# constantinpape/torch-em

Measured on AMD Instinct MI355X. Metric: voxels/sec fwd+bwd, UNet3d 1x128^3 bs=2, higher is better.
Workload: dtype f32-class (forward convs on normalised activations: fp32 operands split into 2 fp16 terms = 22 mantissa bits, lo plane scaled by 2^12 with its own fp32 accumulator, 3 fp16 MFMAs per product; other forward convs 3 bf16 terms / 6 MFMAs; data-gradient convs 2 bf16 terms / 3 MFMAs (16-bit products); WEI

## Files before the change

### torch_em_amd/csrc/conv1x1_stream.hip

```cpp
#include "tem_common.h"
#include "tem_act.h"
#include "conv_split.h"
#include "conv_internal.h"
#include "conv_arith.h"

template <int NS, bool F16, int CT, typename T>
__global__ __launch_bounds__(256) void k_conv1x1_stream(const T* __restrict__ x, int64_t x_ld,
                                                        const unsigned short* __restrict__ wp,
                                                        const float* __restrict__ bias, T* __restrict__ y,
                                                        int64_t y_ld, const T* __restrict__ ref, int64_t ref_ld,
                                                        int64_t NV, int Cin, int Cout, int act, int64_t nmt,
                                                        unsigned* __restrict__ amax) {
    const int lane = threadIdx.x & 63, wv = threadIdx.x >> 6;
    float amx = 0.f;
    const int r = lane & 31, kh = lane >> 5;
    const int ctg = blockIdx.y;
    const int nks = Cin >> 4;
    const uint4* wfrag = reinterpret_cast<const uint4*>(wp) + lane;
    for (int64_t mt = (int64_t)blockIdx.x * 4 + wv; mt < nmt; mt += (int64_t)gridDim.x * 4) {
        const int64_t v = mt * 32 + r;
        const bool vok = v < NV;
        const T* xr = x + (vok ? v : 0) * x_ld + kh * 8;
        floatx16 acc[CT];
#pragma unroll
        for (int ct = 0; ct < CT; ++ct)
#pragma unroll
            for (int k = 0; k < 16; ++k) acc[ct][k] = 0.f;
        for (int ks = 0; ks < nks; ++ks) {
            uint4 t[NS];
            if constexpr (sizeof(T) == 2) {
                static_assert(sizeof(T) == 4 || NS == 1, "16-bit storage: one-term modes only");
                t[0] = make_uint4(0u, 0u, 0u, 0u);
                if (vok) t[0] = *reinterpret_cast<const uint4*>(xr + ks * 16);
            } else {
                float4 a0 = make_float4(0.f, 0.f, 0.f, 0.f), a1 = a0;
                if (vok) {
                    a0 = act_ld4(xr + ks * 16);
                    a1 = act_ld4(xr + ks * 16 + 4);
                }
                float rem[8] = {a0.x, a0.y, a0.z, a0.w, a1.x, a1.y, a1.z, a1.w};
#pragma unroll
                for (int p = 0; p < NS; ++p) {
                    unsigned wds[4];
#pragma unroll
                    for (int e = 0; e < 4; ++e) {
                        const unsigned h = pk16<F16>(rem[2 * e], rem[2 * e + 1]);
                        wds[e] = h;
                        if (p + 1 < NS) {
                            rem[2 * e] -= lo16<F16>(h);
                            rem[2 * e + 1] -= hi16<F16>(h);
                        }
                    }
                    t[p] = make_uint4(wds[0], wds[1], wds[2], wds[3]);
                }
            }
#pragma unroll
            for (int ct = 0; ct < CT; ++ct) {
                const int nt = ctg * CT + ct;
                if (nt * 32 < Cout) {
                    const uint4* f = wfrag + ((int64_t)(nt * nks + ks) * NS) * 64;
                    uint4 b[NS];
#pragma unroll
                    for (int p = 0; p < NS; ++p) b[p] = f[p * 64];
#pragma unroll
                    for (int o = NS - 1; o >= 0; --o)
#pragma unroll
                        for (int i = 0; i <= o; ++i) acc[ct] = mfma16<F16>(b[o - i], t[i], acc[ct]);
                }
            }
        }
        if (vok) {
#pragma unroll
            for (int ct = 0; ct < CT; ++ct) {
#pragma unroll
                for (int q4 = 0; q4 < 4; ++q4) {
                    const int co = (ctg * CT + ct) * 32 + 8 * q4 + 4 * kh;
                    if (co < Cout) {
                        float4 o = make_float4(acc[ct][4 * q4], acc[ct][4 * q4 + 1], acc[ct][4 * q4 + 2], acc[ct][4 * q4 + 3]);
                        if (bias) {
                            const float4 b4 = *reinterpret_cast<const float4*>(bias + co);
                            o.x += b4.x;
                            o.y += b4.y;
                            o.z += b4.z;
                            o.w += b4.w;
                        }
                        o.x = act_apply_b(o.x, act);
                        o.y = act_apply_b(o.y, act);
                        o.z = act_apply_b(o.z, act);
                        o.w = act_apply_b(o.w, act);
                        if (ref) {
                            const float4 rv = act_ld4(ref + v * ref_ld + co);
                            o.x = rv.x > 0.f ? o.x : 0.f;
                            o.y = rv.y > 0.f ? o.y : 0.f;
                            o.z = rv.z > 0.f ? o.z : 0.f;
                            o.w = rv.w > 0.f ? o.w : 0.f;
                        }
                        act_st4(y + v * y_ld + co, o);
                        amx = tem_amax4(amx, o.x, o.y, o.z, o.w);
                    }
                }
            }
        }
    }
    if (amax) tem_amax_commit(amax, amx);
}

template <int NS, bool F16, typename T>
static void stream_launch(const TemConvCall& c, const T* x, int64_t x_ld, const float* wp, const float* bias, T* y, int64_t y_ld,
                          const T* ref, int64_t ref_ld, int64_t NV, int Cin, int Cout, int act, hipStream_t s) {
    const int64_t nmt = (NV + 31) / 32;
    const int ntile = Cout / 32;
    const int CT = ntile >= 2 ? 2 : 1;
    const int ngroups = (ntile + CT - 1) / CT;
    int64_t gx = (nmt + 3) / 4;
    if (gx > 8192) gx = 8192;
    const dim3 grid((unsigned)gx, (unsigned)ngroups);
    unsigned* const amax = c.take_output_amax();
    if (CT == 2)
        hipLaunchKernelGGL((k_conv1x1_stream<NS, F16, 2, T>), grid, dim3(256), 0, s, x, x_ld, (const unsigned short*)wp, bias, y, y_ld,
                           ref, ref_ld, NV, Cin, Cout, act, nmt, amax);
    else
        hipLaunchKernelGGL((k_conv1x1_stream<NS, F16, 1, T>), grid, dim3(256), 0, s, x, x_ld, (const unsigned short*)wp, bias, y, y_ld,
                           ref, ref_ld, NV, Cin, Cout, act, nmt, amax);
}

void tem_conv1x1_stream(const TemConvCall& c, const float* x, int64_t x_ld, const float* wp, const float* bias, float* y, int64_t y_ld,
                        const float* ref, int64_t ref_ld, const TemConvShape& sh, int act, int mode, hipStream_t s) {
    const int st = c.stx, Cin = sh.Cin, Cout = sh.Cout;
    const int64_t NV = sh.NV();
    auto go = [&](auto ns, auto f16, auto t) {
        using T = decltype(t);
        stream_launch<ns(), f16(), T>(c, (const T*)x, x_ld, wp, bias, (T*)y, y_ld, (const T*)ref, ref_ld, NV, Cin, Cout, act, s);
    };
    const TemArith& a = tem_arith(mode);
    if (st == TEM_ST_F16) go(TemInt<1>{}, TemBool<true>{}, tem_f16{});
    else if (st == TEM_ST_BF16) go(TemInt<1>{}, TemBool<false>{}, tem_bf16{});
    else if (a.planes == 3) go(TemInt<3>{}, TemBool<false>{}, float{});
    else if (a.planes == 2) go(TemInt<2>{}, TemBool<false>{}, float{});
    else tem_select_bool(a.elem == TEM_EL_F16, [&](auto f16) { go(TemInt<1>{}, f16, float{}); });
}
```

### torch_em_amd/csrc/dice.hip

```cpp
#include "tem_common.h"

#define DICE_MAX_BLOCKS 2048

extern "C" int64_t tem_dice_ws(int N, int64_t V, int C) {
    (void)N;
    (void)V;
    return (int64_t)DICE_MAX_BLOCKS * C * 4 * (int64_t)sizeof(float);
}

__device__ __forceinline__ float dice_sigmoid(float x) { return 1.f / (1.f + expf(-x)); }

template <bool CFAST>
__global__ void k_dice_partial(const float* __restrict__ p, int64_t p_sn, int64_t p_sc, int64_t p_sv,
                               const float* __restrict__ t, int64_t t_sn, int64_t t_sc, int64_t t_sv,
                               const float* __restrict__ mask, int N, int C, int64_t V, int rows, int64_t vper,
                               int nblk_per_n, float* __restrict__ part, int flags) {
    extern __shared__ float sh[];
    const int NS = (flags & TEM_DICE_BCE) ? 4 : 3;
    const int n = blockIdx.x / nblk_per_n, b = blockIdx.x % nblk_per_n;
    int c, r;
    if (CFAST) {
        c = threadIdx.x % C;
        r = threadIdx.x / C;
    } else {
        r = threadIdx.x % rows;
        c = threadIdx.x / rows;
    }
    int64_t v0 = (int64_t)b * vper, v1 = v0 + vper;
    if (v1 > V) v1 = V;
    const float* pp = p + (int64_t)n * p_sn + (int64_t)c * p_sc;
    const float* tp = t + (int64_t)n * t_sn + (int64_t)c * t_sc;
    const float* mp = mask ? mask + (int64_t)n * t_sn + (int64_t)c * t_sc : nullptr;
    float s0 = 0.f, s1 = 0.f, s2 = 0.f, s3 = 0.f;
    for (int64_t v = v0 + r; v < v1; v += rows) {
        float pv = pp[v * p_sv], tv = tp[v * t_sv];
        if (flags) {
            const float xv = pv;
            if (flags & TEM_DICE_LOGITS) pv = dice_sigmoid(xv);
            if (flags & TEM_DICE_BCE) {
                if (flags & TEM_DICE_LOGITS)
                    s3 += fmaxf(xv, 0.f) - xv * tv + log1pf(expf(-fabsf(xv)));
                else
                    s3 -= tv * fmaxf(logf(pv), -100.f) + (1.f - tv) * fmaxf(logf(1.f - pv), -100.f);
            }
        }
        if (mp) {
            float m = mp[v * t_sv];
            pv *= m;
            tv *= m;
        }
        s0 = fmaf(pv, tv, s0);
        s1 = fmaf(pv, pv, s1);
        s2 = fmaf(tv, tv, s2);
    }
    float* my = sh + ((int64_t)r * C + c) * NS;
    my[0] = s0;
    my[1] = s1;
    my[2] = s2;
    if (NS == 4) my[3] = s3;
    __syncthreads();
    if (r == 0) {
        float a0 = 0.f, a1 = 0.f, a2 = 0.f, a3 = 0.f;
        for (int rr = 0; rr < rows; ++rr) {
            const float* o = sh + ((int64_t)rr * C + c) * NS;
            a0 += o[0];
            a1 += o[1];
            a2 += o[2];
            if (NS == 4) a3 += o[3];
        }
        float* o = part + ((int64_t)blockIdx.x * C + c) * NS;
        o[0] = a0;
        o[1] = a1;
        o[2] = a2;
        if (NS == 4) o[3] = a3;
    }
}

#define DICE_VOX_C 16
template <int VECP>
__global__ __launch_bounds__(256) void k_dice_partial_vox(const float* __restrict__ p, int64_t p_sn, int64_t p_sc, int64_t p_sv,
                                                          const float* __restrict__ t, int64_t t_sn, int64_t t_sc, int64_t t_sv,
                                                          const float* __restrict__ mask, int N, int C, int64_t V, int64_t vper,
                                                          int nblk_per_n, float* __restrict__ part, int flags) {
    __shared__ float shv[4][DICE_VOX_C][4];
    const int NS = (flags & TEM_DICE_BCE) ? 4 : 3;
    const int n = blockIdx.x / nblk_per_n, b = blockIdx.x % nblk_per_n;
    (void)vper;
    const float* pn = p + (int64_t)n * p_sn;
    const float* tn = t + (int64_t)n * t_sn;
    const float* mn = mask ? mask + (int64_t)n * t_sn : nullptr;
    float s0[DICE_VOX_C], s1[DICE_VOX_C], s2[DICE_VOX_C], s3[DICE_VOX_C];
#pragma unroll
    for (int c = 0; c < DICE_VOX_C; ++c) s0[c] = s1[c] = s2[c] = s3[c] = 0.f;
    for (int64_t vb = (int64_t)b * 256 + threadIdx.x; vb < V; vb += (int64_t)nblk_per_n * 256) {
        float pq[DICE_VOX_C], tq[DICE_VOX_C], mq[DICE_VOX_C];
        const float* pv_ = pn + vb * p_sv;
        if constexpr (VECP == 4) {
#pragma unroll
            for (int c = 0; c < DICE_VOX_C; c += 4)
                if (c < C) {
                    const float4 q = *reinterpret_cast<const float4*>(pv_ + c);
                    pq[c] = q.x; pq[c + 1] = q.y; pq[c + 2] = q.z; pq[c + 3] = q.w;
                }
        } else if constexpr (VECP == 2) {
            const float2 q = *reinterpret_cast<const float2*>(pv_);
            pq[0] = q.x; pq[1] = q.y;
        } else {
#pragma unroll
            for (int c = 0; c < DICE_VOX_C; ++c)
                if (c < C) pq[c] = pv_[c * p_sc];
        }
#pragma unroll
        for (int c = 0; c < DICE_VOX_C; ++c)
            if (c < C) {
                tq[c] = tn[c * t_sc + vb * t_sv];
                mq[c] = mn ? mn[c * t_sc + vb * t_sv] : 1.f;
            }
#pragma unroll
        for (int c = 0; c < DICE_VOX_C; ++c)
            if (c < C) {
                float pv = pq[c], tv = tq[c];
                if (flags) {
                    const float xv = pv;
                    if (flags & TEM_DICE_LOGITS) pv = dice_sigmoid(xv);
                    if (flags & TEM_DICE_BCE) {
                        if (flags & TEM_DICE_LOGITS)
                            s3[c] += fmaxf(xv, 0.f) - xv * tv + log1pf(expf(-fabsf(xv)));
                        else
                            s3[c] -= tv * fmaxf(logf(pv), -100.f) + (1.f - tv) * fmaxf(logf(1.f - pv), -100.f);
                    }
                }
                if (mn) {
                    pv *= mq[c];
                    tv *= mq[c];
                }
                s0[c] = fmaf(pv, tv, s0[c]);
                s1[c] = fmaf(pv, pv, s1[c]);
                s2[c] = fmaf(tv, tv, s2[c]);
            }
    }
    const int wv = threadIdx.x >> 6, lane = threadIdx.x & 63;
#pragma unroll
    for (int c = 0; c < DICE_VOX_C; ++c)
        if (c < C) {
            const float a0 = tem_wave_sum(s0[c]), a1 = tem_wave_sum(s1[c]), a2 = tem_wave_sum(s2[c]);
            const float a3 = NS == 4 ? tem_wave_sum(s3[c]) : 0.f;
            if (lane == 0) {
                shv[wv][c][0] = a0;
                shv[wv][c][1] = a1;
                shv[wv][c][2] = a2;
                shv[wv][c][3] = a3;
            }
        }
    __syncthreads();
    for (int i = threadIdx.x; i < C * NS; i += 256) {
        const int c = i / NS, k = i % NS;
        part[((int64_t)blockIdx.x * C + c) * NS + k] = shv[0][c][k] + shv[1][c][k] + shv[2][c][k] + shv[3][c][k];
    }
}

__global__ __launch_bounds__(256) void k_dice_reduce(const float* __restrict__ part, int nblk, int C,
                                                     double* __restrict__ sums, int NS) {
    const int c = blockIdx.x;
    double a[4] = {0.0, 0.0, 0.0, 0.0};
    for (int b = threadIdx.x; b < nblk; b += 256) {
        const float* o = part + ((int64_t)b * C + c) * NS;
        a[0] += (double)o[0];
        a[1] += (double)o[1];
        a[2] += (double)o[2];
        if (NS == 4) a[3] += (double)o[3];
    }
    __shared__ double sh[4][4];
#pragma unroll
    for (int k = 0; k < 4; ++k) {
        a[k] = tem_wave_sum_d(a[k]);
        if ((threadIdx.x & 63) == 0) sh[k][threadIdx.x >> 6] = a[k];
    }
    __syncthreads();
    if (threadIdx.x < NS) sums[c * NS + threadIdx.x] = sh[threadIdx.x][0] + sh[threadIdx.x][1] + sh[threadIdx.x][2] + sh[threadIdx.x][3];
}

static int dice_sums_impl(const float* p, int64_t p_sn, int64_t p_sc, int64_t p_sv, const float* t, int64_t t_sn,
                          int64_t t_sc, int64_t t_sv, const float* mask, int N, int C, int64_t V, double* sums,
                          void* ws, int64_t ws_bytes, int flags, tem_stream_t stream) {
    TEM_REQUIRE(p && t && sums && ws, "tem_dice_sums: null pointer");
    TEM_REQUIRE((flags & ~(TEM_DICE_LOGITS | TEM_DICE_BCE)) == 0 && (!(flags & TEM_DICE_BCE) || !mask),
                "tem_dice_sums2: unknown flags, or the BCE term together with a mask");
    const int NS = (flags & TEM_DICE_BCE) ? 4 : 3;
    TEM_REQUIRE(N > 0 && C > 0 && C <= 1024 && V > 0, "tem_dice_sums: bad shape (C=%d)", C);
    if (ws_bytes < tem_dice_ws(N, V, C)) {
        tem_set_error("tem_dice_sums: workspace too small");
        return TEM_EWS;
    }
    int rows = 256 / C;
    if (rows < 1) rows = 1;
    if (C <= DICE_VOX_C && tem_option(TEM_OPT_DICE_VOX)) rows = 256;
    int threads = C <= DICE_VOX_C && tem_option(TEM_OPT_DICE_VOX) ? 256 : rows * C;
    int64_t nb = tem_cdiv(V, (int64_t)rows * 8);
    int64_t maxb = DICE_MAX_BLOCKS / N;
    if (maxb < 1) {
        tem_set_error("tem_dice_sums: batch too large (N=%d)", N);
        return TEM_EINVAL;
    }
    if (nb > maxb) nb = maxb;
    int64_t vper = tem_cdiv(V, nb);
    int nblk = (int)nb * N;
    size_t lds = (size_t)rows * C * NS * sizeof(float);
    float* part = (float*)ws;
    bool cfast = (p_sc == 1);
    if (C <= DICE_VOX_C && tem_option(TEM_OPT_DICE_VOX)) {
        const bool al = cfast && p_sn % 4 == 0 && p_sv % 4 == 0 && ((uintptr_t)p % 16 == 0);
        if (al && C % 4 == 0)
            hipLaunchKernelGGL((k_dice_partial_vox<4>), dim3(nblk), dim3(256), 0, (hipStream_t)stream, p, p_sn, p_sc, p_sv, t, t_sn,
                               t_sc, t_sv, mask, N, C, V, vper, (int)nb, part, flags);
        else if (cfast && C == 2 && p_sn % 2 == 0 && p_sv == 2 && ((uintptr_t)p % 8 == 0))
            hipLaunchKernelGGL((k_dice_partial_vox<2>), dim3(nblk), dim3(256), 0, (hipStream_t)stream, p, p_sn, p_sc, p_sv, t, t_sn,
                               t_sc, t_sv, mask, N, C, V, vper, (int)nb, part, flags);
        else
            hipLaunchKernelGGL((k_dice_partial_vox<1>), dim3(nblk), dim3(256), 0, (hipStream_t)stream, p, p_sn, p_sc, p_sv, t, t_sn,
                               t_sc, t_sv, mask, N, C, V, vper, (int)nb, part, flags);
    } else if (cfast)
        hipLaunchKernelGGL((k_dice_partial<true>), dim3(nblk), dim3(threads), lds, (hipStream_t)stream, p, p_sn, p_sc,
                           p_sv, t, t_sn, t_sc, t_sv, mask, N, C, V, rows, vper, (int)nb, part, flags);
    else
        hipLaunchKernelGGL((k_dice_partial<false>), dim3(nblk), dim3(threads), lds, (hipStream_t)stream, p, p_sn, p_sc,
                           p_sv, t, t_sn, t_sc, t_sv, mask, N, C, V, rows, vper, (int)nb, part, flags);
    hipLaunchKernelGGL(k_dice_reduce, dim3(C), dim3(256), 0, (hipStream_t)stream, part, nblk, C, sums, NS);
    TEM_CHECK_LAUNCH("tem_dice_sums");
    return TEM_OK;
}

extern "C" int tem_dice_sums(const float* p, int64_t p_sn, int64_t p_sc, int64_t p_sv, const float* t, int64_t t_sn,
                             int64_t t_sc, int64_t t_sv, const float* mask, int N, int C, int64_t V, double* sums,
                             void* ws, int64_t ws_bytes, tem_stream_t stream) {
    return dice_sums_impl(p, p_sn, p_sc, p_sv, t, t_sn, t_sc, t_sv, mask, N, C, V, sums, ws, ws_bytes, 0, stream);
}

extern "C" int tem_dice_sums2(const float* p, int64_t p_sn, int64_t p_sc, int64_t p_sv, const float* t, int64_t t_sn,
                              int64_t t_sc, int64_t t_sv, int N, int C, int64_t V, double* sums, void* ws,
                              int64_t ws_bytes, int flags, tem_stream_t stream) {
    return dice_sums_impl(p, p_sn, p_sc, p_sv, t, t_sn, t_sc, t_sv, nullptr, N, C, V, sums, ws, ws_bytes, flags, stream);
}

__global__ void k_dice_finalize(const double* __restrict__ sums, int C, double eps, int channelwise, int invert,
                                int reduce, float* __restrict__ out, float* __restrict__ ca, float* __restrict__ cb, int NS) {
    if (threadIdx.x != 0 || blockIdx.x != 0) return;
    const double sgn = invert ? -1.0 : 1.0;
    if (!channelwise) {
        double num = 0.0, den = 0.0;
        for (int c = 0; c < C; ++c) {
            num += sums[c * NS];
            den += sums[c * NS + 1] + sums[c * NS + 2];
        }
        double cd = den < eps ? eps : den;
        double score = 2.0 * num / cd;
        out[0] = (float)(invert ? 1.0 - score : score);
        double a = sgn * 2.0 / cd, b = (den >= eps) ? -sgn * 4.0 * num / (cd * cd) : 0.0;
        for (int c = 0; c < C; ++c) {
            ca[c] = (float)a;
            cb[c] = (float)b;
        }
        return;
    }
    double acc = 0.0;
    int arg = 0;
    double best = 0.0;
    for (int c = 0; c < C; ++c) {
        double num = sums[c * NS], den = sums[c * NS + 1] + sums[c * NS + 2];
        double cd = den < eps ? eps : den;
        double score = 2.0 * num / cd;
        double val = invert ? 1.0 - score : score;
        ca[c] = (float)(sgn * 2.0 / cd);
        cb[c] = (float)((den >= eps) ? -sgn * 4.0 * num / (cd * cd) : 0.0);
        if (reduce == 0) out[c] = (float)val;
        acc += val;
        if (c == 0 || (reduce == 3 && val > best) || (reduce == 4 && val < best)) {
            best = val;
            arg = c;
        }
    }
    if (reduce == 1) out[0] = (float)acc;
    if (reduce == 2) {
        out[0] = (float)(acc / C);
        for (int c = 0; c < C; ++c) {
            ca[c] /= (float)C;
            cb[c] /= (float)C;
        }
    }
    if (reduce == 3 || reduce == 4) {
        out[0] = (float)best;
        for (int c = 0; c < C; ++c)
            if (c != arg) {
                ca[c] = 0.f;
                cb[c] = 0.f;
            }
    }
}

static int dice_finalize_impl(const double* sums, int C, double eps, int channelwise, int invert, int reduce, float* out,
                              float* ca, float* cb, int NS, tem_stream_t stream) {
    TEM_REQUIRE(sums && out && ca && cb && C > 0, "tem_dice_finalize: bad arguments");
    TEM_REQUIRE(reduce >= 0 && reduce <= 4, "tem_dice_finalize: Unsupported channel reduction %d", reduce);
    hipLaunchKernelGGL(k_dice_finalize, dim3(1), dim3(64), 0, (hipStream_t)stream, sums, C, eps, channelwise, invert,
                       reduce, out, ca, cb, NS);
    TEM_CHECK_LAUNCH("tem_dice_finalize");
    return TEM_OK;
}
extern "C" int tem_dice_finalize(const double* sums, int C, double eps, int channelwise, int invert, int reduce,
                                 float* out, float* ca, float* cb, tem_stream_t stream) {
    return dice_finalize_impl(sums, C, eps, channelwise, invert, reduce, out, ca, cb, 3, stream);
}
extern "C" int tem_dice_finalize2(const double* sums, int ncol, int C, double eps, int channelwise, int invert, int reduce,
                                  float* out, float* ca, float* cb, tem_stream_t stream) {
    TEM_REQUIRE(ncol == 3 || ncol == 4, "tem_dice_finalize2: ncol must be 3 or 4");
    return dice_finalize_impl(sums, C, eps, channelwise, invert, reduce, out, ca, cb, ncol, stream);
}

template <bool CFAST>
__global__ __launch_bounds__(256) void k_dice_grad(const float* __restrict__ p, int64_t p_sn, int64_t p_sc,
                                                   int64_t p_sv, const float* __restrict__ t, int64_t t_sn,
                                                   int64_t t_sc, int64_t t_sv, const float* __restrict__ mask,
                                                   const float* __restrict__ ca, const float* __restrict__ cb,
                                                   const float* __restrict__ gout, int gout_per_channel,
                                                   float* __restrict__ gp, int64_t g_sn, int64_t g_sc, int64_t g_sv,
                                                   int C, int64_t V, int flags, float w_dice, float w_bce) {
    const int n = blockIdx.y;
    const int64_t items = V * C;
    for (int64_t i = (int64_t)blockIdx.x * 256 + threadIdx.x; i < items; i += (int64_t)gridDim.x * 256) {
        int c;
        int64_t v;
        if (CFAST) {
            v = i / C;
            c = (int)(i - v * C);
        } else {
            c = (int)(i / V);
            v = i - (int64_t)c * V;
        }
        float pv = p[(int64_t)n * p_sn + (int64_t)c * p_sc + v * p_sv];
        float tv = t[(int64_t)n * t_sn + (int64_t)c * t_sc + v * t_sv];
        float m = 1.f;
        if (mask) {
            m = mask[(int64_t)n * t_sn + (int64_t)c * t_sc + v * t_sv];
            pv *= m;
            tv *= m;
        }
        float go = gout ? gout[gout_per_channel ? c : 0] : 1.f;
        if (flags) {
            const float xv = pv;
            if (flags & TEM_DICE_LOGITS) pv = dice_sigmoid(xv);
            float d = w_dice * (ca[c] * tv + cb[c] * pv);
            if (flags & TEM_DICE_LOGITS) d *= pv * (1.f - pv);
            if (flags & TEM_DICE_BCE)
                d += w_bce * ((flags & TEM_DICE_LOGITS) ? (pv - tv) : (pv - tv) / fmaxf(pv * (1.f - pv), 1e-12f));
            gp[(int64_t)n * g_sn + (int64_t)c * g_sc + v * g_sv] = go * d;
            continue;
        }
        gp[(int64_t)n * g_sn + (int64_t)c * g_sc + v * g_sv] = go * (ca[c] * tv + cb[c] * pv) * m;
    }
}

template <int VECP>
__global__ __launch_bounds__(256) void k_dice_grad_vox(const float* __restrict__ p, int64_t p_sn, int64_t p_sc, int64_t p_sv,
                                                       const float* __restrict__ t, int64_t t_sn, int64_t t_sc, int64_t t_sv,
                                                       const float* __restrict__ mask, const float* __restrict__ ca,
                                                       const float* __restrict__ cb, const float* __restrict__ gout,
                                                       int gout_per_channel, float* __restrict__ gp, int64_t g_sn, int64_t g_sc,
                                                       int64_t g_sv, int C, int64_t V, int flags, float w_dice, float w_bce) {
    const int n = blockIdx.y;
    const float* pn = p + (int64_t)n * p_sn;
    const float* tn = t + (int64_t)n * t_sn;
    const float* mn = mask ? mask + (int64_t)n * t_sn : nullptr;
    float* gn = gp + (int64_t)n * g_sn;
    for (int64_t v = (int64_t)blockIdx.x * 256 + threadIdx.x; v < V; v += (int64_t)gridDim.x * 256) {
        float pq[DICE_VOX_C], tq[DICE_VOX_C], mq[DICE_VOX_C], gq[DICE_VOX_C];
        const float* pv_ = pn + v * p_sv;
        if constexpr (VECP == 4) {
#pragma unroll
            for (int c = 0; c < DICE_VOX_C; c += 4)
                if (c < C) {
                    const float4 q = *reinterpret_cast<const float4*>(pv_ + c);
                    pq[c] = q.x; pq[c + 1] = q.y; pq[c + 2] = q.z; pq[c + 3] = q.w;
                }
        } else if constexpr (VECP == 2) {
            const float2 q = *reinterpret_cast<const float2*>(pv_);
            pq[0] = q.x; pq[1] = q.y;
        } else {
#pragma unroll
            for (int c = 0; c < DICE_VOX_C; ++c)
                if (c < C) pq[c] = pv_[c * p_sc];
        }
#pragma unroll
        for (int c = 0; c < DICE_VOX_C; ++c)
            if (c < C) {
                tq[c] = tn[c * t_sc + v * t_sv];
                mq[c] = mn ? mn[c * t_sc + v * t_sv] : 1.f;
            }
#pragma unroll
        for (int c = 0; c < DICE_VOX_C; ++c)
            if (c < C) {
                float pv = pq[c], tv = tq[c];
                const float m = mq[c];
                if (mn) {
                    pv *= m;
                    tv *= m;
                }
                const float go = gout ? gout[gout_per_channel ? c : 0] : 1.f;
                if (flags) {
                    const float xv = pv;
                    if (flags & TEM_DICE_LOGITS) pv = dice_sigmoid(xv);
                    float d = w_dice * (ca[c] * tv + cb[c] * pv);
                    if (flags & TEM_DICE_LOGITS) d *= pv * (1.f - pv);
                    if (flags & TEM_DICE_BCE)
                        d += w_bce * ((flags & TEM_DICE_LOGITS) ? (pv - tv) : (pv - tv) / fmaxf(pv * (1.f - pv), 1e-12f));
                    gq[c] = go * d;
                } else {
                    gq[c] = go * (ca[c] * tv + cb[c] * pv) * m;
                }
            }
        float* gv_ = gn + v * g_sv;
        if constexpr (VECP == 4) {
#pragma unroll
            for (int c = 0; c < DICE_VOX_C; c += 4)
                if (c < C) *reinterpret_cast<float4*>(gv_ + c) = make_float4(gq[c], gq[c + 1], gq[c + 2], gq[c + 3]);
        } else if constexpr (VECP == 2) {
            *reinterpret_cast<float2*>(gv_) = make_float2(gq[0], gq[1]);
        } else {
#pragma unroll
            for (int c = 0; c < DICE_VOX_C; ++c)
                if (c < C) gv_[c * g_sc] = gq[c];
        }
    }
}

static int dice_grad_impl(const float* p, int64_t p_sn, int64_t p_sc, int64_t p_sv, const float* t, int64_t t_sn,
                          int64_t t_sc, int64_t t_sv, const float* mask, const float* ca, const float* cb,
                          const float* gout, int gout_per_channel, float* gp, int64_t g_sn, int64_t g_sc,
                          int64_t g_sv, int N, int C, int64_t V, int flags, float w_dice, float w_bce, tem_stream_t stream) {
    TEM_REQUIRE(p && t && ca && cb && gp && N > 0 && C > 0 && V > 0, "tem_dice_grad: bad arguments");
    TEM_REQUIRE((flags & ~(TEM_DICE_LOGITS | TEM_DICE_BCE)) == 0 && (!flags || !mask), "tem_dice_grad2: unknown flags, or flags with a mask");
    dim3 grid(tem_grid_1d(V * C, 256, 2048), N);
    if (C <= DICE_VOX_C && tem_option(TEM_OPT_DICE_VOX)) {
        const dim3 vgrid(tem_grid_1d(V, 256, 4096), N);
        const bool cl = p_sc == 1 && g_sc == 1;
        const bool al4 = cl && C % 4 == 0 && p_sn % 4 == 0 && p_sv % 4 == 0 && g_sn % 4 == 0 && g_sv % 4 == 0 &&
                         ((uintptr_t)p % 16 == 0) && ((uintptr_t)gp % 16 == 0);
        const bool al2 = cl && C == 2 && p_sv == 2 && g_sv == 2 && p_sn % 2 == 0 && g_sn % 2 == 0 && ((uintptr_t)p % 8 == 0) &&
                         ((uintptr_t)gp % 8 == 0);
#define TEM_DGV(VP)                                                                                                            \
    hipLaunchKernelGGL((k_dice_grad_vox<VP>), vgrid, dim3(256), 0, (hipStream_t)stream, p, p_sn, p_sc, p_sv, t, t_sn, t_sc, t_sv, \
                       mask, ca, cb, gout, gout_per_channel, gp, g_sn, g_sc, g_sv, C, V, flags, w_dice, w_bce)
        if (al4) TEM_DGV(4);
        else if (al2) TEM_DGV(2);
        else TEM_DGV(1);
#undef TEM_DGV
    } else if (p_sc == 1)
        hipLaunchKernelGGL((k_dice_grad<true>), grid, dim3(256), 0, (hipStream_t)stream, p, p_sn, p_sc, p_sv, t, t_sn,
                           t_sc, t_sv, mask, ca, cb, gout, gout_per_channel, gp, g_sn, g_sc, g_sv, C, V, flags, w_dice, w_bce);
    else
        hipLaunchKernelGGL((k_dice_grad<false>), grid, dim3(256), 0, (hipStream_t)stream, p, p_sn, p_sc, p_sv, t, t_sn,
                           t_sc, t_sv, mask, ca, cb, gout, gout_per_channel, gp, g_sn, g_sc, g_sv, C, V, flags, w_dice, w_bce);
    TEM_CHECK_LAUNCH("tem_dice_grad");
    return TEM_OK;
}
extern "C" int tem_dice_grad(const float* p, int64_t p_sn, int64_t p_sc, int64_t p_sv, const float* t, int64_t t_sn,
                             int64_t t_sc, int64_t t_sv, const float* mask, const float* ca, const float* cb,
                             const float* gout, int gout_per_channel, float* gp, int64_t g_sn, int64_t g_sc,
                             int64_t g_sv, int N, int C, int64_t V, tem_stream_t stream) {
    return dice_grad_impl(p, p_sn, p_sc, p_sv, t, t_sn, t_sc, t_sv, mask, ca, cb, gout, gout_per_channel, gp, g_sn, g_sc,
                          g_sv, N, C, V, 0, 1.f, 0.f, stream);
}
extern "C" int tem_dice_grad2(const float* p, int64_t p_sn, int64_t p_sc, int64_t p_sv, const float* t, int64_t t_sn,
                              int64_t t_sc, int64_t t_sv, const float* ca, const float* cb, const float* gout,
                              int gout_per_channel, float* gp, int64_t g_sn, int64_t g_sc, int64_t g_sv, int N, int C,
                              int64_t V, int flags, float w_dice, float w_bce, tem_stream_t stream) {
    return dice_grad_impl(p, p_sn, p_sc, p_sv, t, t_sn, t_sc, t_sv, nullptr, ca, cb, gout, gout_per_channel, gp, g_sn,
                          g_sc, g_sv, N, C, V, flags, w_dice, w_bce, stream);
}
```

Measured before the change: 281.2 million.

## Stage 1x1 conv tiles through LDS with prefetch; unroll dice kernels for C=2

```diff
diff --git a/torch_em_amd/csrc/conv1x1_stream.hip b/torch_em_amd/csrc/conv1x1_stream.hip
--- a/torch_em_amd/csrc/conv1x1_stream.hip
+++ b/torch_em_amd/csrc/conv1x1_stream.hip
@@ -4,81 +4,148 @@
 #include "conv_internal.h"
 #include "conv_arith.h"
 
+#define ST_PITCH 9
+__device__ __forceinline__ void st_lds_fence() { asm volatile("" ::: "memory"); }
+
+struct StLines { uint4 v[4]; };
+template <typename T>
+__device__ __forceinline__ StLines st_load_x(const T* __restrict__ x, int64_t x_ld, int64_t mt, int s, int lr, int lp, int npc, int64_t NV) {
+    StLines o;
+    const int pc = min(s * 8 + lp, npc - 1);
+#pragma unroll
+    for (int j = 0; j < 4; ++j) {
+        const int64_t v = min(mt * 32 + lr + 8 * j, NV - 1);
+        o.v[j] = reinterpret_cast<const uint4*>(x + v * x_ld)[pc];
+    }
+    return o;
+}
+
+template <typename T> struct StRef { typedef act_u2 raw; };
+template <> struct StRef<float> { typedef float4 raw; };
+__device__ __forceinline__ float4 st_ref4(const float*, float4 u) { return u; }
+template <typename T> __device__ __forceinline__ float4 st_ref4(const T*, act_u2 u) {
+    return make_float4(act_lo<T>(u.x), act_hi<T>(u.x), act_lo<T>(u.y), act_hi<T>(u.y));
+}
+
 template <int NS, bool F16, int CT, typename T>
-__global__ __launch_bounds__(256) void k_conv1x1_stream(const T* __restrict__ x, int64_t x_ld,
+__global__ __launch_bounds__(256) __attribute__((amdgpu_waves_per_eu(sizeof(T) == 4 ? 3 : 2))) void k_conv1x1_stream(const T* __restrict__ x, int64_t x_ld,
                                                         const unsigned short* __restrict__ wp,
                                                         const float* __restrict__ bias, T* __restrict__ y,
                                                         int64_t y_ld, const T* __restrict__ ref, int64_t ref_ld,
                                                         int64_t NV, int Cin, int Cout, int act, int64_t nmt,
                                                         unsigned* __restrict__ amax) {
+    static_assert(sizeof(T) == 4 || NS == 1, "16-bit storage: one-term modes only");
+    constexpr int PK = sizeof(T) / 2;
+    constexpr int KPS = 4 / PK;
+    __shared__ uint4 tiles[4][32 * ST_PITCH];
     const int lane = threadIdx.x & 63, wv = threadIdx.x >> 6;
+    uint4* const tl = tiles[wv];
     float amx = 0.f;
     const int r = lane & 31, kh = lane >> 5;
+    const int lr = lane >> 3, lp = lane & 7;
     const int ctg = blockIdx.y;
     const int nks = Cin >> 4;
+    const int npc = nks * 2 * PK;
+    const int nst = (nks + KPS - 1) / KPS;
     const uint4* wfrag = reinterpret_cast<const uint4*>(wp) + lane;
+    float4 bs[CT];
+#pragma unroll
+    for (int ct = 0; ct < CT; ++ct) {
+        const int co = (ctg * CT + ct) * 32 + 4 * lp;
+        bs[ct] = make_float4(0.f, 0.f, 0.f, 0.f);
+        if (bias && co < Cout) bs[ct] = *reinterpret_cast<const float4*>(bias + co);
+    }
     for (int64_t mt = (int64_t)blockIdx.x * 4 + wv; mt < nmt; mt += (int64_t)gridDim.x * 4) {
-        const int64_t v = mt * 32 + r;
-        const bool vok = v < NV;
-        const T* xr = x + (vok ? v : 0) * x_ld + kh * 8;
-        floatx16 acc[CT];
-#pragma unroll
-        for (int ct = 0; ct < CT; ++ct)
-#pragma unroll
-            for (int k = 0; k < 16; ++k) acc[ct][k] = 0.f;
-        for (int ks = 0; ks < nks; ++ks) {
-            uint4 t[NS];
-            if constexpr (sizeof(T) == 2) {
-                static_assert(sizeof(T) == 4 || NS == 1, "16-bit storage: one-term modes only");
-                t[0] = make_uint4(0u, 0u, 0u, 0u);
-                if (vok) t[0] = *reinterpret_cast<const uint4*>(xr + ks * 16);
-            } else {
-                float4 a0 = make_float4(0.f, 0.f, 0.f, 0.f), a1 = a0;
-                if (vok) {
-                    a0 = act_ld4(xr + ks * 16);
-                    a1 = act_ld4(xr + ks * 16 + 4);
-                }
-                float rem[8] = {a0.x, a0.y, a0.z, a0.w, a1.x, a1.y, a1.z, a1.w};
-#pragma unroll
-                for (int p = 0; p < NS; ++p) {
-                    unsigned wds[4];
-#pragma unroll
-                    for (int e = 0; e < 4; ++e) {
-                        const unsigned h = pk16<F16>(rem[2 * e], rem[2 * e + 1]);
-                        wds[e] = h;
-                        if (p + 1 < NS) {
-                            rem[2 * e] -= lo16<F16>(h);
-                            rem[2 * e + 1] -= hi16<F16>(h);
-                        }
-                    }
-                    t[p] = make_uint4(wds[0], wds[1], wds[2], wds[3]);
-                }
-            }
+        StLines xs = st_load_x(x, x_ld, mt, 0, lr, lp, npc, NV);
+        typename StRef<T>::raw rf[CT][4];
+        if (ref) {
 #pragma unroll
             for (int ct = 0; ct < CT; ++ct) {
-                const int nt = ctg * CT + ct;
-                if (nt * 32 < Cout) {
-                    const uint4* f = wfrag + ((int64_t)(nt * nks + ks) * NS) * 64;
-                    uint4 b[NS];
-#pragma unroll
-                    for (int p = 0; p < NS; ++p) b[p] = f[p * 64];
-#pragma unroll
-                    for (int o = NS - 1; o >= 0; --o)
-#pragma unroll
-                        for (int i = 0; i <= o; ++i) acc[ct] = mfma16<F16>(b[o - i], t[i], acc[ct]);
+                const int co = (ctg * CT + ct) * 32 + 4 * lp;
+                if (co < Cout) {
+#pragma unroll
+                    for (int j = 0; j < 4; ++j) rf[ct][j] = *reinterpret_cast<const typename StRef<T>::raw*>(ref + min(mt * 32 + lr + 8 * j, NV - 1) * ref_ld + co);
                 }
             }
         }
-        if (vok) {
-#pragma unroll
-            for (int ct = 0; ct < CT; ++ct) {
+        floatx16 acc[CT];
+#pragma unroll
+        for (int ct = 0; ct < CT; ++ct)
+#pragma unroll
+            for (int k = 0; k < 16; ++k) acc[ct][k] = 0.f;
+        for (int s = 0; s < nst; ++s) {
+#pragma unroll
+            for (int j = 0; j < 4; ++j) tl[(lr + 8 * j) * ST_PITCH + lp] = xs.v[j];
+            st_lds_fence();
+            if (s + 1 < nst) xs = st_load_x(x, x_ld, mt, s + 1, lr, lp, npc, NV);
+#pragma unroll
+            for (int kk = 0; kk < KPS; ++kk) {
+                const int ks = s * KPS + kk;
+                if (ks < nks) {
+                    uint4 b[CT][NS];
+#pragma unroll
+                    for (int ct = 0; ct < CT; ++ct) {
+                        const int nt = ctg * CT + ct;
+                        if (nt * 32 < Cout) {
+                            const uint4* f = wfrag + ((int64_t)(nt * nks + ks) * NS) * 64;
+#pragma unroll
+                            for (int p = 0; p < NS; ++p) b[ct][p] = f[p * 64];
+                        }
+                    }
+                    const uint4* pr = tl + r * ST_PITCH + (kk * 2 + kh) * PK;
+                    uint4 t[NS];
+                    if constexpr (sizeof(T) == 2) {
+                        t[0] = pr[0];
+                    } else {
+                        const uint4 u0 = pr[0], u1 = pr[1];
+                        float rem[8] = {__uint_as_float(u0.x), __uint_as_float(u0.y), __uint_as_float(u0.z), __uint_as_float(u0.w),
+                                        __uint_as_float(u1.x), __uint_as_float(u1.y), __uint_as_float(u1.z), __uint_as_float(u1.w)};
+#pragma unroll
+                        for (int p = 0; p < NS; ++p) {
+                            unsigned wds[4];
+#pragma unroll
+                            for (int e = 0; e < 4; ++e) {
+                                const unsigned h = pk16<F16>(rem[2 * e], rem[2 * e + 1]);
+                                wds[e] = h;
+                                if (p + 1 < NS) {
+                                    rem[2 * e] -= lo16<F16>(h);
+                                    rem[2 * e + 1] -= hi16<F16>(h);
+                                }
+                            }
+                            t[p] = make_uint4(wds[0], wds[1], wds[2], wds[3]);
+                        }
+                    }
+#pragma unroll
+                    for (int ct = 0; ct < CT; ++ct) {
+                        if ((ctg * CT + ct) * 32 < Cout) {
+#pragma unroll
+                            for (int o = NS - 1; o >= 0; --o)
+#pragma unroll
+                                for (int i = 0; i <= o; ++i) acc[ct] = mfma16<F16>(b[ct][o - i], t[i], acc[ct]);
+                        }
+                    }
+                }
+            }
+            st_lds_fence();
+        }
+#pragma unroll
+        for (int ct = 0; ct < CT; ++ct) {
+            const int co = (ctg * CT + ct) * 32 + 4 * lp;
+            if ((ctg * CT + ct) * 32 < Cout) {
 #pragma unroll
                 for (int q4 = 0; q4 < 4; ++q4) {
-                    const int co = (ctg * CT + ct) * 32 + 8 * q4 + 4 * kh;
-                    if (co < Cout) {
-                        float4 o = make_float4(acc[ct][4 * q4], acc[ct][4 * q4 + 1], acc[ct][4 * q4 + 2], acc[ct][4 * q4 + 3]);
+                    const float a0 = acc[ct][4 * q4], a1 = acc[ct][4 * q4 + 1], a2 = acc[ct][4 * q4 + 2], a3 = acc[ct][4 * q4 + 3];
+                    tl[r * ST_PITCH + 2 * q4 + kh] = make_uint4(__float_as_uint(a0), __float_as_uint(a1), __float_as_uint(a2), __float_as_uint(a3));
+                }
+                st_lds_fence();
+                const float4 b4 = bs[ct];
+#pragma unroll
+                for (int j = 0; j < 4; ++j) {
+                    const int64_t v = mt * 32 + lr + 8 * j;
+                    const uint4 u = tl[(lr + 8 * j) * ST_PITCH + lp];
+                    if (v < NV && co < Cout) {
+                        float4 o = make_float4(__uint_as_float(u.x), __uint_as_float(u.y), __uint_as_float(u.z), __uint_as_float(u.w));
                         if (bias) {
-                            const float4 b4 = *reinterpret_cast<const float4*>(bias + co);
                             o.x += b4.x;
                             o.y += b4.y;
                             o.z += b4.z;
@@ -89,7 +156,7 @@
                         o.z = act_apply_b(o.z, act);
                         o.w = act_apply_b(o.w, act);
                         if (ref) {
-                            const float4 rv = act_ld4(ref + v * ref_ld + co);
+                            const float4 rv = st_ref4(ref, rf[ct][j]);
                             o.x = rv.x > 0.f ? o.x : 0.f;
                             o.y = rv.y > 0.f ? o.y : 0.f;
                             o.z = rv.z > 0.f ? o.z : 0.f;
@@ -99,6 +166,7 @@
                         amx = tem_amax4(amx, o.x, o.y, o.z, o.w);
                     }
                 }
+                st_lds_fence();
             }
         }
     }
diff --git a/torch_em_amd/csrc/dice.hip b/torch_em_amd/csrc/dice.hip
--- a/torch_em_amd/csrc/dice.hip
+++ b/torch_em_amd/csrc/dice.hip
@@ -89,59 +89,69 @@
     const float* pn = p + (int64_t)n * p_sn;
     const float* tn = t + (int64_t)n * t_sn;
     const float* mn = mask ? mask + (int64_t)n * t_sn : nullptr;
-    float s0[DICE_VOX_C], s1[DICE_VOX_C], s2[DICE_VOX_C], s3[DICE_VOX_C];
-#pragma unroll
-    for (int c = 0; c < DICE_VOX_C; ++c) s0[c] = s1[c] = s2[c] = s3[c] = 0.f;
-    for (int64_t vb = (int64_t)b * 256 + threadIdx.x; vb < V; vb += (int64_t)nblk_per_n * 256) {
-        float pq[DICE_VOX_C], tq[DICE_VOX_C], mq[DICE_VOX_C];
-        const float* pv_ = pn + vb * p_sv;
-        if constexpr (VECP == 4) {
-#pragma unroll
-            for (int c = 0; c < DICE_VOX_C; c += 4)
+    constexpr int CM = VECP == 2 ? 2 : DICE_VOX_C, U = VECP == 2 ? 4 : 1;
+    float s0[CM], s1[CM], s2[CM], s3[CM];
+#pragma unroll
+    for (int c = 0; c < CM; ++c) s0[c] = s1[c] = s2[c] = s3[c] = 0.f;
+    const int64_t vstep = (int64_t)nblk_per_n * 256;
+    for (int64_t vb0 = (int64_t)b * 256 + threadIdx.x; vb0 < V; vb0 += U * vstep) {
+        float pq[U][CM], tq[U][CM], mq[U][CM];
+#pragma unroll
+        for (int u = 0; u < U; ++u) {
+            const int64_t vb = min(vb0 + u * vstep, V - 1);
+            const float* pv_ = pn + vb * p_sv;
+            if constexpr (VECP == 4) {
+#pragma unroll
+                for (int c = 0; c < CM; c += 4)
+                    if (c < C) {
+                        const float4 q = *reinterpret_cast<const float4*>(pv_ + c);
+                        pq[u][c] = q.x; pq[u][c + 1] = q.y; pq[u][c + 2] = q.z; pq[u][c + 3] = q.w;
+                    }
+            } else if constexpr (VECP == 2) {
+                const float2 q = *reinterpret_cast<const float2*>(pv_);
+                pq[u][0] = q.x; pq[u][1] = q.y;
+            } else {
+#pragma unroll
+                for (int c = 0; c < CM; ++c)
+                    if (c < C) pq[u][c] = pv_[c * p_sc];
+            }
+#pragma unroll
+            for (int c = 0; c < CM; ++c)
                 if (c < C) {
-                    const float4 q = *reinterpret_cast<const float4*>(pv_ + c);
-                    pq[c] = q.x; pq[c + 1] = q.y; pq[c + 2] = q.z; pq[c + 3] = q.w;
+                    tq[u][c] = tn[c * t_sc + vb * t_sv];
+                    mq[u][c] = mn ? mn[c * t_sc + vb * t_sv] : 1.f;
                 }
-        } else if constexpr (VECP == 2) {
-            const float2 q = *reinterpret_cast<const float2*>(pv_);
-            pq[0] = q.x; pq[1] = q.y;
-        } else {
-#pragma unroll
-            for (int c = 0; c < DICE_VOX_C; ++c)
-                if (c < C) pq[c] = pv_[c * p_sc];
-        }
-#pragma unroll
-        for (int c = 0; c < DICE_VOX_C; ++c)
-            if (c < C) {
-                tq[c] = tn[c * t_sc + vb * t_sv];
-                mq[c] = mn ? mn[c * t_sc + vb * t_sv] : 1.f;
-            }
-#pragma unroll
-        for (int c = 0; c < DICE_VOX_C; ++c)
-            if (c < C) {
-                float pv = pq[c], tv = tq[c];
-                if (flags) {
-                    const float xv = pv;
-                    if (flags & TEM_DICE_LOGITS) pv = dice_sigmoid(xv);
-                    if (flags & TEM_DICE_BCE) {
-                        if (flags & TEM_DICE_LOGITS)
-                            s3[c] += fmaxf(xv, 0.f) - xv * tv + log1pf(expf(-fabsf(xv)));
-                        else
-                            s3[c] -= tv * fmaxf(logf(pv), -100.f) + (1.f - tv) * fmaxf(logf(1.f - pv), -100.f);
+        }
+#pragma unroll
+        for (int u = 0; u < U; ++u) {
+            const bool ok = vb0 + u * vstep < V;
+#pragma unroll
+            for (int c = 0; c < CM; ++c)
+                if (c < C) {
+                    float pv = pq[u][c], tv = tq[u][c];
+                    if (flags) {
+                        const float xv = pv;
+                        if (flags & TEM_DICE_LOGITS) pv = dice_sigmoid(xv);
+                        if (flags & TEM_DICE_BCE) {
+                            if (flags & TEM_DICE_LOGITS)
+                                s3[c] = ok ? s3[c] + (fmaxf(xv, 0.f) - xv * tv + log1pf(expf(-fabsf(xv)))) : s3[c];
+                            else
+                                s3[c] = ok ? s3[c] - (tv * fmaxf(logf(pv), -100.f) + (1.f - tv) * fmaxf(logf(1.f - pv), -100.f)) : s3[c];
+                        }
                     }
+                    if (mn) {
+                        pv *= mq[u][c];
+                        tv *= mq[u][c];
+                    }
+                    s0[c] = ok ? fmaf(pv, tv, s0[c]) : s0[c];
+                    s1[c] = ok ? fmaf(pv, pv, s1[c]) : s1[c];
+                    s2[c] = ok ? fmaf(tv, tv, s2[c]) : s2[c];
                 }
-                if (mn) {
-                    pv *= mq[c];
-                    tv *= mq[c];
-                }
-                s0[c] = fmaf(pv, tv, s0[c]);
-                s1[c] = fmaf(pv, pv, s1[c]);
-                s2[c] = fmaf(tv, tv, s2[c]);
-            }
+        }
     }
     const int wv = threadIdx.x >> 6, lane = threadIdx.x & 63;
 #pragma unroll
-    for (int c = 0; c < DICE_VOX_C; ++c)
+    for (int c = 0; c < CM; ++c)
         if (c < C) {
             const float a0 = tem_wave_sum(s0[c]), a1 = tem_wave_sum(s1[c]), a2 = tem_wave_sum(s2[c]);
             const float a3 = NS == 4 ? tem_wave_sum(s3[c]) : 0.f;
@@ -371,63 +381,75 @@
     const float* tn = t + (int64_t)n * t_sn;
     const float* mn = mask ? mask + (int64_t)n * t_sn : nullptr;
     float* gn = gp + (int64_t)n * g_sn;
-    for (int64_t v = (int64_t)blockIdx.x * 256 + threadIdx.x; v < V; v += (int64_t)gridDim.x * 256) {
-        float pq[DICE_VOX_C], tq[DICE_VOX_C], mq[DICE_VOX_C], gq[DICE_VOX_C];
-        const float* pv_ = pn + v * p_sv;
-        if constexpr (VECP == 4) {
-#pragma unroll
-            for (int c = 0; c < DICE_VOX_C; c += 4)
+    constexpr int CM = VECP == 2 ? 2 : DICE_VOX_C, U = VECP == 2 ? 4 : 1;
+    const int64_t vstep = (int64_t)gridDim.x * 256;
+    for (int64_t v0 = (int64_t)blockIdx.x * 256 + threadIdx.x; v0 < V; v0 += U * vstep) {
+        float pq[U][CM], tq[U][CM], mq[U][CM];
+#pragma unroll
+        for (int u = 0; u < U; ++u) {
+            const int64_t v = min(v0 + u * vstep, V - 1);
+            const float* pv_ = pn + v * p_sv;
+            if constexpr (VECP == 4) {
+#pragma unroll
+                for (int c = 0; c < CM; c += 4)
+                    if (c < C) {
+                        const float4 q = *reinterpret_cast<const float4*>(pv_ + c);
+                        pq[u][c] = q.x; pq[u][c + 1] = q.y; pq[u][c + 2] = q.z; pq[u][c + 3] = q.w;
+                    }
+            } else if constexpr (VECP == 2) {
+                const float2 q = *reinterpret_cast<const float2*>(pv_);
+                pq[u][0] = q.x; pq[u][1] = q.y;
+            } else {
+#pragma unroll
+                for (int c = 0; c < CM; ++c)
+                    if (c < C) pq[u][c] = pv_[c * p_sc];
+            }
+#pragma unroll
+            for (int c = 0; c < CM; ++c)
                 if (c < C) {
-                    const float4 q = *reinterpret_cast<const float4*>(pv_ + c);
-                    pq[c] = q.x; pq[c + 1] = q.y; pq[c + 2] = q.z; pq[c + 3] = q.w;
+                    tq[u][c] = tn[c * t_sc + v * t_sv];
+                    mq[u][c] = mn ? mn[c * t_sc + v * t_sv] : 1.f;
                 }
-        } else if constexpr (VECP == 2) {
-            const float2 q = *reinterpret_cast<const float2*>(pv_);
-            pq[0] = q.x; pq[1] = q.y;
-        } else {
-#pragma unroll
-            for (int c = 0; c < DICE_VOX_C; ++c)
-                if (c < C) pq[c] = pv_[c * p_sc];
-        }
-#pragma unroll
-        for (int c = 0; c < DICE_VOX_C; ++c)
-            if (c < C) {
-                tq[c] = tn[c * t_sc + v * t_sv];
-                mq[c] = mn ? mn[c * t_sc + v * t_sv] : 1.f;
+        }
+#pragma unroll
+        for (int u = 0; u < U; ++u) {
+            const int64_t v = v0 + u * vstep;
+            if (v >= V) break;
+            float gq[CM];
+#pragma unroll
+            for (int c = 0; c < CM; ++c)
+                if (c < C) {
+                    float pv = pq[u][c], tv = tq[u][c];
+                    const float m = mq[u][c];
+                    if (mn) {
+                        pv *= m;
+                        tv *= m;
+                    }
+                    const float go = gout ? gout[gout_per_channel ? c : 0] : 1.f;
+                    if (flags) {
+                        const float xv = pv;
+                        if (flags & TEM_DICE_LOGITS) pv = dice_sigmoid(xv);
+                        float d = w_dice * (ca[c] * tv + cb[c] * pv);
+                        if (flags & TEM_DICE_LOGITS) d *= pv * (1.f - pv);
+                        if (flags & TEM_DICE_BCE)
+                            d += w_bce * ((flags & TEM_DICE_LOGITS) ? (pv - tv) : (pv - tv) / fmaxf(pv * (1.f - pv), 1e-12f));
+                        gq[c] = go * d;
+                    } else {
+                        gq[c] = go * (ca[c] * tv + cb[c] * pv) * m;
+                    }
+                }
+            float* gv_ = gn + v * g_sv;
+            if constexpr (VECP == 4) {
+#pragma unroll
+                for (int c = 0; c < CM; c += 4)
+                    if (c < C) *reinterpret_cast<float4*>(gv_ + c) = make_float4(gq[c], gq[c + 1], gq[c + 2], gq[c + 3]);
+            } else if constexpr (VECP == 2) {
+                *reinterpret_cast<float2*>(gv_) = make_float2(gq[0], gq[1]);
+            } else {
+#pragma unroll
+                for (int c = 0; c < CM; ++c)
+                    if (c < C) gv_[c * g_sc] = gq[c];
             }
-#pragma unroll
-        for (int c = 0; c < DICE_VOX_C; ++c)
-            if (c < C) {
-                float pv = pq[c], tv = tq[c];
-                const float m = mq[c];
-                if (mn) {
-                    pv *= m;
-                    tv *= m;
-                }
-                const float go = gout ? gout[gout_per_channel ? c : 0] : 1.f;
-                if (flags) {
-                    const float xv = pv;
-                    if (flags & TEM_DICE_LOGITS) pv = dice_sigmoid(xv);
-                    float d = w_dice * (ca[c] * tv + cb[c] * pv);
-                    if (flags & TEM_DICE_LOGITS) d *= pv * (1.f - pv);
-                    if (flags & TEM_DICE_BCE)
-                        d += w_bce * ((flags & TEM_DICE_LOGITS) ? (pv - tv) : (pv - tv) / fmaxf(pv * (1.f - pv), 1e-12f));
-                    gq[c] = go * d;
-                } else {
-                    gq[c] = go * (ca[c] * tv + cb[c] * pv) * m;
-                }
-            }
-        float* gv_ = gn + v * g_sv;
-        if constexpr (VECP == 4) {
-#pragma unroll
-            for (int c = 0; c < DICE_VOX_C; c += 4)
-                if (c < C) *reinterpret_cast<float4*>(gv_ + c) = make_float4(gq[c], gq[c + 1], gq[c + 2], gq[c + 3]);
-        } else if constexpr (VECP == 2) {
-            *reinterpret_cast<float2*>(gv_) = make_float2(gq[0], gq[1]);
-        } else {
-#pragma unroll
-            for (int c = 0; c < DICE_VOX_C; ++c)
-                if (c < C) gv_[c * g_sc] = gq[c];
         }
     }
 }
```

Result: no change. 282.8 million, median of 6 (+0.6%).
